# jypjypjypjyp/lvio_fusion

Hardware: AMD Instinct MI355X
Metric: local-BA iters/sec (50 KF x 10k pts) + ICP Mpairs/sec (higher is better)
Workload: dtype f64; 1 GPU; configs[3]: full sliding-window LM iteration, 50 keyframes x 10 000 landmarks (10000 TwoCamera + 71789 TwoFrame + 9629 PoseOnly + 49 IMU factors), device-resident LM loop, one independent window per GPU; n_kf=50, n_lm=10000, parallelism=1 independent windows

## Files before the change

### lvio_fusion_amd/csrc/lvf_internal.hpp

```cpp
#pragma once
#include <hip/hip_runtime.h>
#include <algorithm>
#include <cstdarg>
#include <cstdint>
#include <cstdlib>
#include <cstdio>
#include <cstring>
#include <memory>
#include <mutex>
#include <string>
#include <unordered_map>
#include <utility>
#include <vector>

#include "../../include/lvf.h"
#include "lvf_math.hpp"

namespace lvf {

void set_error(const char* fmt, ...);
int hip_fail(hipError_t e, const char* what, const char* file, int line);

#define LVF_HIP(call)                                                          \
  do {                                                                         \
// ... 356 lines not shown
  lvf::DevBuf<double> corr;
  lvf::DevBuf<char> icp_dev;
  lvf::HostPin<char> icp_host;
  lvf::DevBuf<float> create_src; lvf::HostPin<float> create_stage; hipEvent_t create_done = nullptr;
  ~lvf_scan() { if (create_done) { (void)hipEventSynchronize(create_done); (void)hipEventDestroy(create_done); } }
};

struct lvf_cloud {
  lvf_ctx* ctx = nullptr;
  int n = 0;
  lvf::DevBuf<float4> pts;
};

struct lvf_problem;
namespace lvf {
template <int CTRL>
__device__ __forceinline__ double quad_perm(double v) {
  const int lo = __builtin_amdgcn_mov_dpp(__double2loint(v), CTRL, 0xF, 0xF, true);
  const int hi = __builtin_amdgcn_mov_dpp(__double2hiint(v), CTRL, 0xF, 0xF, true);
  return __hiloint2double(hi, lo);
}
__device__ __forceinline__ double quad_sum(double v) {
  v += quad_perm<0xB1>(v);
  v += quad_perm<0x4E>(v);
  return v;
}

__device__ __forceinline__ double lane_bcast(double v, int srclane) {
  const int lo = __builtin_amdgcn_readlane(__double2loint(v), srclane);
  const int hi = __builtin_amdgcn_readlane(__double2hiint(v), srclane);
  return __hiloint2double(hi, lo);
}
__device__ __forceinline__ int wave_incl_scan(int v) {
  v += __builtin_amdgcn_update_dpp(0, v, 0x111, 0xF, 0xF, true);
  v += __builtin_amdgcn_update_dpp(0, v, 0x112, 0xF, 0xF, true);
  v += __builtin_amdgcn_update_dpp(0, v, 0x114, 0xF, 0xF, true);
  v += __builtin_amdgcn_update_dpp(0, v, 0x118, 0xF, 0xF, true);
  v += __builtin_amdgcn_update_dpp(0, v, 0x142, 0xA, 0xF, false);
  v += __builtin_amdgcn_update_dpp(0, v, 0x143, 0xC, 0xF, false);
  return v;
}
__device__ __forceinline__ double row16_sum(double v) {
  v = quad_sum(v);
  v += quad_perm<0x141>(v);
  v += quad_perm<0x140>(v);
  return v;
}
__device__ __forceinline__ double wave_sum(double v) {
  v = quad_sum(v);
  v += quad_perm<0x141>(v);
  v += quad_perm<0x140>(v);
  return (lane_bcast(v, 0) + lane_bcast(v, 16)) + (lane_bcast(v, 32) + lane_bcast(v, 48));
}
typedef unsigned lvf_v2u __attribute__((ext_vector_type(2)));
__device__ __forceinline__ void swap_halves32(double& x, double& y) {
  const lvf_v2u lo = __builtin_amdgcn_permlane32_swap((unsigned)__double2loint(x), (unsigned)__double2loint(y), false, false);
  const lvf_v2u hi = __builtin_amdgcn_permlane32_swap((unsigned)__double2hiint(x), (unsigned)__double2hiint(y), false, false);
  x = __hiloint2double((int)hi.x, (int)lo.x); y = __hiloint2double((int)hi.y, (int)lo.y);
}
__device__ __forceinline__ void swap_rows16(double& x, double& y) {
  const lvf_v2u lo = __builtin_amdgcn_permlane16_swap((unsigned)__double2loint(x), (unsigned)__double2loint(y), false, false);
  const lvf_v2u hi = __builtin_amdgcn_permlane16_swap((unsigned)__double2hiint(x), (unsigned)__double2hiint(y), false, false);
  x = __hiloint2double((int)hi.x, (int)lo.x); y = __hiloint2double((int)hi.y, (int)lo.y);
}
__device__ __forceinline__ double wave_sum32(double v[32]) {
  const int lane = threadIdx.x & 63;
#pragma unroll
  for (int i = 0; i < 16; ++i) { swap_halves32(v[i], v[i + 16]); v[i] += v[i + 16]; }
#pragma unroll
  for (int i = 0; i < 8; ++i) { swap_rows16(v[i], v[i + 8]); v[i] += v[i + 8]; }
  const bool b3 = lane & 8, b2 = lane & 4, b1 = lane & 2;
#pragma unroll
  for (int i = 0; i < 4; ++i) { const double keep = b3 ? v[i + 4] : v[i], send = b3 ? v[i] : v[i + 4]; v[i] = keep + quad_perm<0x128>(send); }
#pragma unroll
  for (int i = 0; i < 2; ++i) { const double keep = b2 ? v[i + 2] : v[i], send = b2 ? v[i] : v[i + 2]; v[i] = keep + quad_perm<0x141>(send); }
  { const double keep = b1 ? v[1] : v[0], send = b1 ? v[0] : v[1]; v[0] = keep + quad_perm<0x4E>(send); }
  return v[0] + quad_perm<0xB1>(v[0]);
}

__device__ __forceinline__ bool cell_runs(int c, int& start, int& len) {
  const int lane = threadIdx.x & 63;
  const int prev = __shfl_up(c, 1);
  const bool head = lane == 0 || c != prev;
  const unsigned long long hm = __ballot(head);
  const unsigned long long upto = (lane == 63) ? ~0ull : ((2ull << lane) - 1ull);
  start = 63 - __clzll((long long)(hm & upto));
  const unsigned long long above = hm & ~upto;
  len = (above ? __ffsll((long long)above) - 1 : 64) - lane;
  return head;
}


int problem_configure(lvf_problem* p);
}
extern "C" __attribute__((visibility("hidden"))) int lvf_problem_solve_then(lvf_problem* p, const lvf_solver_options* o, lvf_solver_summary* summary, int (*tail)(void*), void* user);
namespace lvf {
int device_sort_pairs_u32(lvf_ctx* ctx, const unsigned* keys_in, unsigned* keys_out, const int* vals_in, int* vals_out, int n, int key_bits);
struct SortP { int n, bits, db, nbins; };
constexpr int kSortMaxDigitBits = 11;
struct SortScratch { DevBuf<int> hist; DevBuf<unsigned> tkeys; DevBuf<int> tvals; };
struct SortJobDc {
  hipStream_t q; const unsigned* keys_in; unsigned* keys_out; const int* vals_in; int* vals_out; const SortP* sp; SortScratch* keep;
  const unsigned* ki; const int* vi; unsigned* ko; int* vo;
};
int device_sort_pairs_u32_dc_multi(lvf_ctx* ctx, int n_jobs, SortJobDc* jobs, int cap, int passes);
int device_scan1(lvf_ctx* ctx, const int* in, int cap, const int* n_dev, int* pos, int* total_out, const float4* pts, float4* out);
int device_scan1_on(lvf_ctx* ctx, hipStream_t q, int lane, const int* in, int cap, const int* n_dev, int* pos, int* total_out, const float4* pts, float4* out);
int side_stream(lvf_ctx* ctx, hipStream_t* out);
int enter(lvf_ctx* ctx);
const uint8_t* image_level0(const lvf_image* img, int* width, int* height, lvf_ctx** ctx);
int image_begin(const char* who, lvf_ctx* ctx, int width, int height, int max_level, lvf_image** out, uint8_t** level0);
int image_chain(lvf_image* img);
int device_exclusive_scan_i32(lvf_ctx* ctx, const int* in, int n, int* out);
int compact_points(lvf_ctx* ctx, const float4* pts, int n, const int* flags_dev, lvf_cloud** out);
struct DcTailPlan { bool supported, two_streams; int cap, passes, grid_cells, lane_ground, max_iterations, min_neighbors; float leaf, radius, thr; };
int dc_tail_begin(lvf_ctx* ctx, int cap, float resolution, float max_range, DevBuf<unsigned char>& state, std::shared_ptr<void>& keep, DcTailPlan* plan);
int dc_tail_fork(lvf_ctx* ctx, const DcTailPlan& plan, hipStream_t* q);
int dc_tail_run(lvf_ctx* ctx, const DcTailPlan& plan, hipStream_t q, const float4* surf_raw, const int* n_surf_raw, const float4* ground_raw, const int* n_ground_raw,
                unsigned long long seed, DevBuf<unsigned char>& state, std::shared_ptr<void>& keep, DevBuf<float4>& surf_out, DevBuf<float4>& ground_out);
int dc_state_bytes();
int dc_state_counts_offset();
int transform_points(lvf_ctx* ctx, const float4* in, int n, const double* pose, lvf_cloud** out);
constexpr int kDeskewFastKnots = 8;
struct DeskewRt { double R[9], t[3]; };
struct DeskewP {
  const double* knots; int n, k0, nk;
  double t_lo, t_hi, t0;
  DeskewRt E, A;
};
int deskew_prepare(const char* who, lvf_ctx* ctx, const lvf_trajectory* tr, double frame_time, const double* frame_pose7, double cycle_time, const double* extrinsic7,
// ... 40 lines not shown
```

### lvio_fusion_amd/csrc/solver_kernels.hip

```cpp
#include <hip/hip_ext.h>
#include <algorithm>
#include <chrono>
#include <cmath>
#include <cstdlib>
#include <memory>
#include <unordered_map>

#include "factor_eval.hpp"
#include "prior_eval.hpp"
#include "lvf_internal.hpp"
#include "imu_eval.hpp"

namespace lvf {
struct TfWork;
struct LmCtl;
struct Chain;
struct StageClock;
struct SpNode { int col, row_off, m, id; };
constexpr int kSpMaxLevels = 12, kSpMaxRows = 768;
struct SpLevels { int n; int first[kSpMaxLevels]; int count[kSpMaxLevels]; };
struct JacobiDev { GP<double> h0; GP<const int> frozen; };
struct SpSrc {
  GP<const double> B; int ldB, dp; GP<const double> gc; GP<const double> radius; GP<const int> rows_nat;
  GP<int> wait_counter; int wait_target; GP<int> done_counter;
// ... 217 lines not shown
                                               const uint8_t* __restrict__ pose_const, double* __restrict__ B, int ld,
                                               double* __restrict__ gc, double* __restrict__ E, int ldE,
                                               double* __restrict__ C, double* __restrict__ gr, double* __restrict__ cost) {
  __shared__ PoseD s_pose[kMaxStagedKf];
  stage_poses<kT>(s_pose, s.poses, n_kf);
  const int i = blockIdx.x * kT + threadIdx.x;
  double c = 0.0;
  if (i < n) {
    const int l = lm[i], k1 = kf1[i], k2 = kf2[i];
    const double2 a = fo[i], b = ob[i];
    const PoseD P1 = fetch_pose(s_pose, s.poses, n_kf, k1), P2 = fetch_pose(s_pose, s.poses, n_kf, k2);
    double r[2], Jd[2], L1[12], L2[12];
    if (COST_ONLY) { double J1[14], J2[14]; eval_two_frame<false>(P1, P2, left, right, a.x, a.y, b.x, b.y, s.inv_depth[l], s.w_kf[k2], r, Jd, J1, J2); }
    else eval_two_frame_local(P1, P2, left, right, a.x, a.y, b.x, b.y, s.inv_depth[l], s.w_kf[k2], r, Jd, L1, L2);
    double rho;
    const double sc = robust_scale(huber, r[0] * r[0] + r[1] * r[1], rho);
    c = 0.5 * rho;
    if (!COST_ONLY) {
      {
        const double s1 = (pose_const[k1] & 1) ? 0.0 : sc, s2 = (pose_const[k2] & 1) ? 0.0 : sc;
#pragma unroll
        for (int q = 0; q < 12; ++q) { L1[q] *= s1; L2[q] *= s2; }
      }
      const double r0 = sc * r[0], r1 = sc * r[1], d0 = sc * Jd[0], d1 = sc * Jd[1];
      atomicAdd(&C[l], d0 * d0 + d1 * d1);
      atomicAdd(&gr[l], d0 * r0 + d1 * r1);
      if (k1 == k2) {
#pragma unroll
        for (int q = 0; q < 12; ++q) L1[q] += L2[q];
        add_block66(B, ld, 6 * k1, 6 * k1, L1, L1);
#pragma unroll
        for (int q = 0; q < 6; ++q) { atomicAdd(&gc[6 * k1 + q], L1[q] * r0 + L1[6 + q] * r1); atomicAdd(&E[(size_t)l * ldE + 6 * k1 + q], L1[q] * d0 + L1[6 + q] * d1); }
      } else {
        add_block66(B, ld, 6 * k1, 6 * k1, L1, L1);
        add_block66(B, ld, 6 * k2, 6 * k2, L2, L2);
        if (k2 > k1) add_block66(B, ld, 6 * k2, 6 * k1, L2, L1); else add_block66(B, ld, 6 * k1, 6 * k2, L1, L2);
#pragma unroll
        for (int q = 0; q < 6; ++q) {
          atomicAdd(&gc[6 * k1 + q], L1[q] * r0 + L1[6 + q] * r1);
          atomicAdd(&gc[6 * k2 + q], L2[q] * r0 + L2[6 + q] * r1);
          atomicAdd(&E[(size_t)l * ldE + 6 * k1 + q], L1[q] * d0 + L1[6 + q] * d1);
          atomicAdd(&E[(size_t)l * ldE + 6 * k2 + q], L2[q] * d0 + L2[6 + q] * d1);
        }
      }
    }
  }
  block_add(c, cost);
}

struct TfWork { int first, count, k2; };
struct TfCompact { int on; GP<const int> slot; GP<double> slotB, slabP, slabQ; int staged; };
constexpr int kSlabRow = 64, kSlabQ = 32;
constexpr int kAccSlots = 63;
constexpr int kStageWave = 64 * 9 + 32;
template <bool DYN = false>
__device__ __forceinline__ void lin_tf_sorted_body(const int vb, const TfWork* __restrict__ work, int n_kf, const double2* __restrict__ fo,
                                                      const double2* __restrict__ ob, const int* __restrict__ lm,
                                                      const int* __restrict__ kf1, StateP s, CamD left, CamD right, double huber,
                                                      const uint8_t* __restrict__ pose_const, double* __restrict__ B, int ld,
                                                      double* __restrict__ gc, double* __restrict__ E, int ldE,
                                                      double* __restrict__ C, double* __restrict__ gr, double* __restrict__ cost, int unique_lk2,
                                                      unsigned long long* dbg = nullptr, const TfCompact cp = TfCompact{0, nullptr, nullptr, nullptr, nullptr, 1}, const int dbg_nw = 0) {
  __shared__ PoseD s_pose_st[DYN ? 1 : kMaxStagedKf];
  __shared__ double s_acc_st[DYN ? 1 : kMaxStagedKf * kAccSlots];
  __shared__ double s_k2_st[DYN ? 1 : 27];
  extern __shared__ double lin_lds[];
  PoseD* s_pose = DYN ? reinterpret_cast<PoseD*>(lin_lds) : s_pose_st;
  double* s_acc = DYN ? lin_lds + (sizeof(PoseD) / 8) * n_kf : s_acc_st;
  double* s_k2 = DYN ? s_acc + kAccSlots * n_kf : s_k2_st;
  double* s_stage = DYN ? s_k2 + 32 + (threadIdx.x >> 6) * kStageWave : nullptr;
  int* s_stage_k1 = reinterpret_cast<int*>(s_stage + 64 * 9);
  const TfWork w = work[vb];
  auto mark = [&](int k) { if (dbg && threadIdx.x == 0) dbg[(size_t)vb * 8 + k] = wall_clock64(); };
  unsigned long long* dbgw = dbg ? dbg + (size_t)dbg_nw * 8 + 8 + (size_t)vb * 16 + (threadIdx.x >> 6) * 4 : nullptr;
  auto markw = [&](int k) { if (dbgw && (threadIdx.x & 63) == 0) dbgw[k] = wall_clock64(); };
  mark(0);
  for (int e = threadIdx.x; e < n_kf * kAccSlots; e += kT) s_acc[e] = 0.0;
  if (threadIdx.x < 27) s_k2[threadIdx.x] = 0.0;
  stage_poses<kT>(s_pose, s.poses, n_kf);
  mark(1);
  const int k2 = w.k2;
  double c = 0.0;
  double v[27];
#pragma unroll
  for (int q = 0; q < 27; ++q) v[q] = 0.0;
  const bool active = (int)threadIdx.x < w.count;
  markw(0);
  int k1 = 0;
  double L1[12], L2[12], r0 = 0.0, r1 = 0.0;
#pragma unroll
  for (int q = 0; q < 12; ++q) { L1[q] = 0.0; L2[q] = 0.0; }
  if (active) {
    const int i = w.first + threadIdx.x;
    const int l = lm[i];
    k1 = kf1[i];
    const double2 a = fo[i], b = ob[i];
    double r[2], Jd[2];
    eval_two_frame_local(s_pose[k1], s_pose[k2], left, right, a.x, a.y, b.x, b.y, s.inv_depth[l], s.w_kf[k2], r, Jd, L1, L2);
    double rho;
    const double sc = robust_scale(huber, r[0] * r[0] + r[1] * r[1], rho);
    c = 0.5 * rho;
    {
      const double s1 = (pose_const[k1] & 1) ? 0.0 : sc, s2 = (pose_const[k2] & 1) ? 0.0 : sc;
#pragma unroll
      for (int q = 0; q < 12; ++q) { L1[q] *= s1; L2[q] *= s2; }
    }
    r0 = sc * r[0]; r1 = sc * r[1];
    const double d0 = sc * Jd[0], d1 = sc * Jd[1];
    if (cp.on) {
      double* el = E + (size_t)l * ldE + 6 * k2;
      double2* rec = reinterpret_cast<double2*>(cp.slotB + (size_t)cp.slot[i] * 8);
      double e1[6];
#pragma unroll
      for (int q = 0; q < 6; ++q) { e1[q] = L1[q] * d0 + L1[6 + q] * d1; el[q] = L2[q] * d0 + L2[6 + q] * d1; }
      rec[0] = make_double2(e1[0], e1[1]); rec[1] = make_double2(e1[2], e1[3]); rec[2] = make_double2(e1[4], e1[5]);
      rec[3] = make_double2(d0 * d0 + d1 * d1, d0 * r0 + d1 * r1);
    } else {
      atomicAdd(&C[l], d0 * d0 + d1 * d1);
      atomicAdd(&gr[l], d0 * r0 + d1 * r1);
      double* el = E + (size_t)l * ldE;
#pragma unroll
      for (int q = 0; q < 6; ++q) {
        atomicAdd(&el[6 * k1 + q], L1[q] * d0 + L1[6 + q] * d1);
        const double e2 = L2[q] * d0 + L2[6 + q] * d1;
        if (unique_lk2) el[6 * k2 + q] = e2; else atomicAdd(&el[6 * k2 + q], e2);
      }
    }
  }
  mark(2); markw(1);
  {
    {
      int q = 0;
#pragma unroll
      for (int x = 0; x < 6; ++x)
#pragma unroll
        for (int y = 0; y <= x; ++y) v[q++] = L2[x] * L2[y] + L2[6 + x] * L2[6 + y];
#pragma unroll
      for (int x = 0; x < 6; ++x) v[21 + x] = L2[x] * r0 + L2[6 + x] * r1;
    }
    const int lane = threadIdx.x & 63;
    unsigned long long remaining = __ballot(active);
    bool mine_done = !active;
    int n_groups = 0;
    for (unsigned long long rem = remaining; rem && n_groups < 5; ++n_groups)
      rem &= ~__ballot(active && k1 == __builtin_amdgcn_readlane(k1, (int)__ffsll((long long)rem) - 1));
    const int min_group = n_groups <= 4 ? 1 : 16;
    if (dbgw && lane == 0) dbgw[3] = (unsigned long long)n_groups;
#pragma unroll 1
    for (int round = 0; round < 4 && remaining; ++round) {
      const int k1u = __builtin_amdgcn_readlane(k1, (int)__ffsll((long long)remaining) - 1);
      const bool sel = active && !mine_done && k1 == k1u;
      const unsigned long long m = __ballot(sel);
      if (__popcll(m) < min_group) break;
      double* accu = s_acc + k1u * kAccSlots;
      double z = sel ? 1.0 : 0.0;
      asm volatile("" : "+v"(z));
      double M[12];
#pragma unroll
      for (int i = 0; i < 12; ++i) M[i] = L1[i] * z;
#pragma unroll
      for (int bt = 0; bt < 2; ++bt) {
        double t[32];
#pragma unroll
        for (int i = 0; i < 32; ++i) t[i] = 0.0;
        int q = 0;
#pragma unroll
        for (int x = 0; x < 6; ++x)
#pragma unroll
          for (int y = 0; y <= x; ++y) { if ((q >> 5) == bt) t[q & 31] = M[x] * L1[y] + M[6 + x] * L1[6 + y]; ++q; }
#pragma unroll
        for (int x = 0; x < 6; ++x) { if ((q >> 5) == bt) t[q & 31] = M[x] * r0 + M[6 + x] * r1; ++q; }
#pragma unroll
        for (int x = 0; x < 6; ++x)
#pragma unroll
          for (int y = 0; y < 6; ++y) { if ((q >> 5) == bt) t[q & 31] = L2[x] * M[y] + L2[6 + x] * M[6 + y]; ++q; }
        const double tot = wave_sum32(t);
        const int slot = 32 * bt + (lane >> 1);
        if (!(lane & 1) && slot < 63 && tot != 0.0) atomicAdd(&accu[slot], tot);
      }
      mine_done = mine_done || sel;
      remaining &= ~m;
    }
    if (DYN && n_groups > 4 && cp.staged) {
      double z = (active && !mine_done) ? 1.0 : 0.0;
      asm volatile("" : "+v"(z));
      double M[12];
#pragma unroll
      for (int i = 0; i < 12; ++i) M[i] = L1[i] * z;
      s_stage_k1[lane] = (active && !mine_done) ? k1 : -1;
      const int ss = lane & 7, part = lane >> 3;
      __builtin_amdgcn_fence(__ATOMIC_RELEASE, "wavefront");
      __builtin_amdgcn_wave_barrier();
      __builtin_amdgcn_fence(__ATOMIC_ACQUIRE, "wavefront");
      int kk[9];
#pragma unroll
      for (int j = 0; j < 9; ++j) kk[j] = (8 * part + j < 64) ? s_stage_k1[8 * part + j] : -2;
#pragma unroll
      for (int ch = 0; ch < 8; ++ch) {
        double t[8];
#pragma unroll
        for (int i = 0; i < 8; ++i) t[i] = 0.0;
        int q = 0;
#pragma unroll
        for (int x = 0; x < 6; ++x)
#pragma unroll
          for (int y = 0; y <= x; ++y) { if ((q >> 3) == ch) t[q & 7] = M[x] * L1[y] + M[6 + x] * L1[6 + y]; ++q; }
#pragma unroll
        for (int x = 0; x < 6; ++x) { if ((q >> 3) == ch) t[q & 7] = M[x] * r0 + M[6 + x] * r1; ++q; }
#pragma unroll
        for (int x = 0; x < 6; ++x)
#pragma unroll
          for (int y = 0; y < 6; ++y) { if ((q >> 3) == ch) t[q & 7] = L2[x] * M[y] + L2[6 + x] * M[6 + y]; ++q; }
        __builtin_amdgcn_wave_barrier();
#pragma unroll
        for (int i = 0; i < 8; ++i) s_stage[lane * 9 + i] = t[i];
        __builtin_amdgcn_fence(__ATOMIC_RELEASE, "wavefront");
        __builtin_amdgcn_wave_barrier();
        __builtin_amdgcn_fence(__ATOMIC_ACQUIRE, "wavefront");
        const int slot = 8 * ch + ss;
        double val[8];
#pragma unroll
        for (int j = 0; j < 8; ++j) val[j] = s_stage[(8 * part + j) * 9 + ss];
        double run = 0.0;
#pragma unroll
        for (int j = 0; j < 8; ++j) {
          run += val[j];
          if (j == 7 || kk[j + 1] != kk[j]) {
            if (kk[j] >= 0 && slot < kAccSlots && run != 0.0) atomicAdd(&s_acc[kk[j] * kAccSlots + slot], run);
            run = 0.0;
          }
        }
      }
    } else if (!mine_done) {
      double* acc = s_acc + k1 * kAccSlots;
      int q = 0;
#pragma unroll
      for (int x = 0; x < 6; ++x)
#pragma unroll
        for (int y = 0; y <= x; ++y) atomicAdd(&acc[q++], L1[x] * L1[y] + L1[6 + x] * L1[6 + y]);
#pragma unroll
      for (int x = 0; x < 6; ++x) atomicAdd(&acc[21 + x], L1[x] * r0 + L1[6 + x] * r1);
#pragma unroll
      for (int x = 0; x < 6; ++x)
#pragma unroll
        for (int y = 0; y < 6; ++y) atomicAdd(&acc[27 + 6 * x + y], L2[x] * L1[y] + L2[6 + x] * L1[6 + y]);
    }
  }
  mark(3); markw(2);
  {
    double v32[32];
#pragma unroll
    for (int q = 0; q < 32; ++q) v32[q] = q < 27 ? v[q] : 0.0;
    const double tot = wave_sum32(v32);
    const int lane = threadIdx.x & 63;
    if (!(lane & 1) && (lane >> 1) < 27 && tot != 0.0) atomicAdd(&s_k2[lane >> 1], tot);
  }
  block_add(c, cost);
  __syncthreads();
  mark(4);
  if (cp.on) {
    if (threadIdx.x < kSlabQ) cp.slabQ[(size_t)vb * kSlabQ + threadIdx.x] = threadIdx.x < 27 ? s_k2[threadIdx.x] : 0.0;
    double* P = cp.slabP + (size_t)vb * n_kf * kSlabRow;
    for (int e = threadIdx.x; e < k2 * kSlabRow; e += kT) {
      const int kk = e >> 6, slot = e & 63;
      P[e] = slot < kAccSlots ? s_acc[kk * kAccSlots + slot] : 0.0;
    }
  } else {
  if (threadIdx.x < 27) {
    const double val = s_k2[threadIdx.x];
    if (val != 0.0) {
      if (threadIdx.x < 21) {
        int x = 0, rem = threadIdx.x;
        while (rem > x) { rem -= x + 1; ++x; }
        atomicAdd(&B[(size_t)(6 * k2 + x) * ld + 6 * k2 + rem], val);
      } else atomicAdd(&gc[6 * k2 + threadIdx.x - 21], val);
    }
  }
  for (int e = threadIdx.x; e < n_kf * kAccSlots; e += kT) {
    const double val = s_acc[e];
    if (val == 0.0) continue;
    const int k1 = e / kAccSlots, slot = e % kAccSlots;
    if (slot < 21) {
      int x = 0, rem = slot;
      while (rem > x) { rem -= x + 1; ++x; }
      atomicAdd(&B[(size_t)(6 * k1 + x) * ld + 6 * k1 + rem], val);
    } else if (slot < 27) {
      atomicAdd(&gc[6 * k1 + slot - 21], val);
    } else {
      const int x = (slot - 27) / 6, y = (slot - 27) % 6;
      if (k2 > k1) atomicAdd(&B[(size_t)(6 * k2 + x) * ld + 6 * k1 + y], val);
      else atomicAdd(&B[(size_t)(6 * k1 + y) * ld + 6 * k2 + x], val);
    }
  }
  }
  __syncthreads();
  mark(5);
}
struct CostVisual {
  int n_tc, n_tf, n_po, g_tc, g_tf;
  GP<const double2> tc_lo, tc_ro; GP<const int> tc_lm, tc_kf; GP<const double> tc_w; CamD tc_left, tc_right;
  GP<const double2> tf_fo, tf_ob; GP<const int> tf_lm, tf_k1, tf_k2; CamD tf_left, tf_right;
  GP<const double2> po_ob; GP<const int> po_kf, po_pwi; GP<const double> po_pw; CamD po_cam;
};
struct ImuEvalArgs { int n; GP<const double> pre, sqrt_info; GP<const int> kf_i, kf_j; };
struct CostArgs {
  CostVisual a; int n_kf; StateP s; double huber; GP<double> cost; int nblocks; GP<const int> done;
  ImuEvalArgs imu; int g_imu;
  int tiles;
  ZeroList zero; int zero_wgs;
// ... 346 lines not shown
  if (tid < 64) {
    double c = tid < 15 ? 0.5 * sr[tid] * sr[tid] : 0.0;
    c = wave_sum(c);
    if (tid == 0) atomicAdd(cost + (f & (kStripes - 1)), c);
  }
  for (int e = tid; e < 30 * 30; e += kT) {
    const int a = e / 30, b = e % 30;
    const int ga = sidx[a], gb = sidx[b];
    if (gb > ga || (ga == gb && a != b)) continue;
    double h = 0.0;
#pragma unroll
    for (int k = 0; k < 15; ++k) h += sJ[k * 30 + a] * sJ[k * 30 + b];
    atomicAdd(&B[(size_t)ga * ld + gb], h);
  }
  if (tid < 30) {
    double g = 0.0;
#pragma unroll
    for (int k = 0; k < 15; ++k) g += sJ[k * 30 + tid] * sr[k];
    atomicAdd(&gc[sidx[tid]], g);
  }
  if (dbg) dbg[4] = wall_clock64();
}

struct LinVisual {
  int n_tfw, g_tc;
  GP<const TfWork> work; GP<const double2> tf_fo, tf_ob; GP<const int> tf_lm, tf_k1; CamD tf_left, tf_right; int unique_lk2; TfCompact cp;
  int n_tc; GP<const double2> tc_lo, tc_ro; GP<const int> tc_lm, tc_kf; GP<const double> tc_w; CamD tc_left, tc_right;
  int n_po, g_po; GP<const double2> po_ob; GP<const int> po_kf, po_pwi; GP<const double> po_pw; CamD po_cam;
  int n_imu; GP<const double> imu_res; ImuJ imu_J; GP<const int> imu_i, imu_j; ImuEvalArgs imu;
};
struct LinArgs {
  LinVisual v; int n_kf; StateP s; double huber; GP<const uint8_t> pose_const; GP<double> B; int ld; GP<double> gc; GP<double> E; int ldE; GP<double> C, gr, cost;
  int nblocks; GP<const int> done; GP<unsigned long long> dbg; int rows;
  GP<double> scal_reset;
  AccSel acc;
};
__device__ __forceinline__ void reset_step_scalars(double* scal) {
  for (int k = SC_COST_NEW + threadIdx.x; k < SC_N; k += kT) scal[k] = 0.0;
  if (threadIdx.x == 0) { *reinterpret_cast<int*>(scal + SC_FAIL) = 0; *reinterpret_cast<int*>(scal + SC_TICKET) = 0; }
}
__device__ __forceinline__ void lin_visual_run(const int bx, const LinArgs& A, const int set, const StateP s, double* cost) {
  const LinVisual& a = A.v;
  const int g_imu_first = a.imu.pre ? a.n_imu : 0;
  const int b = bx - g_imu_first;
  const int n_kf = A.n_kf; const double huber = A.huber; const uint8_t* pose_const = A.pose_const;
  auto pick = [set](GP<double> p0, GP<double> p1) -> double* { return (double*)(p0.p + (p1.p - p0.p) * (ptrdiff_t)set); };
  double* B = pick(A.B, A.acc.B); const int ld = A.ld; double* gc = pick(A.gc, A.acc.gc); double* E = pick(A.E, A.acc.E); const int ldE = A.ldE;
  double* C = pick(A.C, A.acc.C); double* gr = pick(A.gr, A.acc.gr);
  TfCompact cp = a.cp;
  cp.slotB = pick(a.cp.slotB, A.acc.slotB);
  if (bx < g_imu_first)
    lin_imu_eval_body(bx, a.imu, n_kf, s, pose_const, B, ld, gc, cost, A.dbg ? A.dbg + (size_t)a.n_tfw * 8 : nullptr);
  else if (b < a.n_tfw)
    lin_tf_sorted_body<true>(b, a.work, n_kf, a.tf_fo, a.tf_ob, a.tf_lm, a.tf_k1, s, a.tf_left, a.tf_right, huber, pose_const, B, ld, gc, E, ldE, C, gr, cost,
                       a.unique_lk2, A.dbg, cp, a.n_tfw);
  else if (b < a.n_tfw + a.g_tc)
    lin_tc_body<false>(b - a.n_tfw, a.n_tc, a.tc_lo, a.tc_ro, a.tc_lm, a.tc_kf, a.tc_w, s, a.tc_left, a.tc_right, huber, C, gr, cost);
  else if (b < a.n_tfw + a.g_tc + a.g_po)
    lin_po_body<false, true>(b - a.n_tfw - a.g_tc, a.n_po, n_kf, a.po_ob, a.po_kf, a.po_pwi, a.po_pw, s, a.po_cam, huber, pose_const, B, ld, gc, cost);
  else
    lin_imu_body4<true>(b - a.n_tfw - a.g_tc - a.g_po, a.n_imu, n_kf, a.imu_res, a.imu_J, a.imu_i, a.imu_j, s.poses, pose_const, B, ld, gc, cost);
}
__device__ __forceinline__ void lin_visual_body(const int bx, const LinArgs& A) {
  if (bx >= A.nblocks || (A.done && *A.done)) return;
  if (bx == 0 && A.scal_reset) reset_step_scalars(A.scal_reset);
  lin_visual_run(bx, A, 0, A.s, A.cost);
}
__global__ __launch_bounds__(kT) __attribute__((amdgpu_waves_per_eu(3))) void k_lin_visual(LinArgs a) { lin_visual_body(blockIdx.x, a); }
__global__ __launch_bounds__(kT) __attribute__((amdgpu_waves_per_eu(3))) void k_lin_visual_b(const LinArgs* __restrict__ t) { lin_visual_body(blockIdx.x, t[blockIdx.y]); }
__global__ __launch_bounds__(kT) __attribute__((amdgpu_waves_per_eu(3))) void k_lin_visual_bt(const LinArgs* __restrict__ t) { lin_visual_body(blockIdx.y, t[blockIdx.x]); }

struct TfReduceArgs {
  int n_kf, n_wg; GP<const int> run_first; GP<const double> slabP, slabQ; GP<double> B; int ld; GP<double> gc; int nblocks; GP<const int> done;
  int own_blocks; SpArgs ride;
  AccSel acc; GP<const int> pending; ZeroList stand0, stand1; int zero_wgs;
};
template <bool SEL>
__device__ __forceinline__ void tf_reduce_body(const int bx0, const TfReduceArgs& A) {
  if (bx0 >= A.nblocks) {
    const int zw = (int)bx0 - A.nblocks;
    if (SEL && zw < A.zero_wgs) {
      if (acc_set(A.acc)) zero_list_share(A.stand0, zw, A.zero_wgs);
      else zero_list_share(A.stand1, zw, A.zero_wgs);
    }
    return;
  }
  if (A.done && *A.done) return;
  if (bx0 < A.ride.nblocks) { sp_ride<SEL>(bx0, A.ride); return; }
  if (SEL && A.pending && !*A.pending) return;
  const bool s1 = acc_set_t<SEL>(A.acc) != 0;
  double* const Bs = s1 ? (double*)A.acc.B : (double*)A.B;
  double* const gcs = s1 ? (double*)A.acc.gc : (double*)A.gc;
  const int bx = bx0 - A.ride.nblocks;
  const int n_kf = A.n_kf;
  const int nchunk = (A.n_wg + 63) / 64;
  if (bx < n_kf * nchunk) {
    __shared__ double part[8][32];
    const int k = bx / nchunk, c = bx - k * nchunk, v = threadIdx.x & 31, g = threadIdx.x >> 5;
    const int r0 = A.run_first[k], r1 = A.run_first[k + 1];
    double acc = 0.0;
    if (v < 27) {
      const double* slabP = A.slabP; const double* slabQ = A.slabQ;
      double t8[8]; bool keep[8];
#pragma unroll
      for (int u = 0; u < 8; ++u) {
        const int wg = 64 * c + g + 8 * u, wgc = min(wg, A.n_wg - 1);
        const bool useP = wgc >= r1;
// ... 2669 lines not shown
  bool imu_done = false;
  const bool clean = !lin || (c.fast && p->accum_clean);
  p->accum_clean = false;
  if (p->clk && p->clk->on) (void)hipEventRecord(p->clk->ev[p->clk->rep][0], q);
  if (!clean) LVF_CHAIN_LAUNCH(p, ST_IMU_LIN, k_zero_multi, dim3(512, c.zero.count), dim3(kT), 0, q, c.zero);
  if (c.fast) {
    imu_done = true;
    stage_mark(p, ST_IMU_LIN, clean ? 0 : 1);
    LinArgs la = c.lin;
    la.huber = huber;
    if (!gated) la.done = nullptr;
    if (!iteration) la.scal_reset = nullptr;
    static const bool lin_timing = std::getenv("LVF_LIN_TIMING") != nullptr;
    if (lin_timing) { LVF_TRY(p->dbg_lin.ensure((size_t)la.v.n_tfw * 24 + 8)); la.dbg = p->dbg_lin.p; }
    static const size_t lds_pad = [] { const char* e = std::getenv("LVF_LIN_LDS_PAD"); return e ? (size_t)std::atoi(e) : (size_t)0; }();
    if (lin) LVF_CHAIN_LAUNCH(p, ST_LIN_VISUAL, k_lin_visual, dim3(la.nblocks), dim3(kT), c.lin_lds + lds_pad, q, la);
    stage_mark(p, ST_LIN_VISUAL, lin ? 1 : 0);
    if (p->compact) {
      TfReduceArgs ra = c.red;
      if (!gated) ra.done = nullptr;
      if (!iteration) { ra.nblocks = ra.own_blocks; ra.ride.nblocks = 0; }
      int zero_wgs = 0;
      if (acc) {
        ra.acc = *acc; acc_patch(ra.ride, acc);
        ra.pending = lin ? nullptr : &p->ctl.p->lin_pending;
        ra.stand0 = c.stand0; ra.stand1 = c.stand1; ra.zero_wgs = zero_wgs = kEndZeroWgs;
      }
      LVF_CHAIN_LAUNCH(p, ST_TF_REDUCE, k_tf_reduce, dim3(ra.nblocks + zero_wgs), dim3(kT), ra.ride.nblocks > 0 ? c.red_lds : 0, q, ra);
    }
    stage_mark(p, ST_TF_REDUCE, p->compact ? 1 : 0);
    if (lin_timing) {
      std::vector<unsigned long long> t((size_t)la.v.n_tfw * 8);
      LVF_HIP(hipStreamSynchronize(q));
      LVF_HIP(hipMemcpy(t.data(), p->dbg_lin.p, t.size() * 8, hipMemcpyDeviceToHost));
      double ph[5] = {0, 0, 0, 0, 0}; unsigned long long first = ~0ull, last = 0, last_start = 0;
      for (int w = 0; w < la.v.n_tfw; ++w) {
        for (int k = 0; k < 5; ++k) ph[k] += (double)(t[(size_t)w * 8 + k + 1] - t[(size_t)w * 8 + k]) * 0.01;
        first = std::min(first, t[(size_t)w * 8]); last = std::max(last, t[(size_t)w * 8 + 5]); last_start = std::max(last_start, t[(size_t)w * 8]);
      }
      {
        double mx[5] = {0, 0, 0, 0, 0}; int slow = 0; double slow_t = 0;
        for (int w = 0; w < la.v.n_tfw; ++w) {
          for (int k = 0; k < 5; ++k) mx[k] = std::max(mx[k], (double)(t[(size_t)w * 8 + k + 1] - t[(size_t)w * 8 + k]) * 0.01);
          const double tot = (double)(t[(size_t)w * 8 + 5] - t[(size_t)w * 8]) * 0.01;
          if (tot > slow_t) { slow_t = tot; slow = w; }
        }
        std::vector<TfWork> hw((size_t)la.v.n_tfw);
        LVF_HIP(hipMemcpy(hw.data(), la.v.work, hw.size() * sizeof(TfWork), hipMemcpyDeviceToHost));
        std::fprintf(stderr, "lin_tf: per-phase MAX over the workgroups (us): %.2f | %.2f | %.2f | %.2f | %.2f ; slowest workgroup %d (k2 = %d, %d blocks): %.2f us =", mx[0], mx[1], mx[2], mx[3], mx[4], slow, hw[slow].k2, hw[slow].count, slow_t);
        for (int k = 0; k < 5; ++k) std::fprintf(stderr, " %.2f", (double)(t[(size_t)slow * 8 + k + 1] - t[(size_t)slow * 8 + k]) * 0.01);
        {
          unsigned long long u[16];
          LVF_HIP(hipMemcpy(u, p->dbg_lin.p + (size_t)la.v.n_tfw * 8 + 8 + (size_t)slow * 16, sizeof(u), hipMemcpyDeviceToHost));
          std::fprintf(stderr, " ; its waves (eval us, k1-sum us, groups):");
          for (int wv = 0; wv < 4; ++wv) std::fprintf(stderr, " [%.2f %.2f %llu]", (double)(u[4 * wv + 1] - u[4 * wv]) * 0.01, (double)(u[4 * wv + 2] - u[4 * wv + 1]) * 0.01, u[4 * wv + 3]);
        }
        std::fprintf(stderr, " ; mean duration by k2 decile:");
        const int nk = la.n_kf;
        for (int dcl = 0; dcl < 5; ++dcl) {
          double sum = 0; int cnt = 0;
          for (int w = 0; w < la.v.n_tfw; ++w) if (hw[w].k2 * 5 / std::max(nk, 1) == dcl) { sum += (double)(t[(size_t)w * 8 + 5] - t[(size_t)w * 8]) * 0.01; ++cnt; }
          std::fprintf(stderr, " %.1f(%d)", cnt ? sum / cnt : 0.0, cnt);
        }
        std::fprintf(stderr, "\n");
      }
      std::fprintf(stderr, "lin_tf: the TwoFrame workgroups START within %.2f us of each other; starts of workgroups 0, 1/4, 1/2, 3/4, last (us after the first): %.2f %.2f %.2f %.2f %.2f\n", (double)(last_start - first) * 0.01,
                   (double)(t[0] - first) * 0.01, (double)(t[(size_t)(la.v.n_tfw / 4) * 8] - first) * 0.01, (double)(t[(size_t)(la.v.n_tfw / 2) * 8] - first) * 0.01,
                   (double)(t[(size_t)(3 * la.v.n_tfw / 4) * 8] - first) * 0.01, (double)(t[(size_t)(la.v.n_tfw - 1) * 8] - first) * 0.01);
      std::fprintf(stderr, "lin_tf phases (us, mean over %d workgroups): stage %.2f | eval+landmark atomics %.2f | k1 sums %.2f | k2 sums %.2f | flush %.2f ; first start -> last end %.2f\n",
                   la.v.n_tfw, ph[0] / la.v.n_tfw, ph[1] / la.v.n_tfw, ph[2] / la.v.n_tfw, ph[3] / la.v.n_tfw, ph[4] / la.v.n_tfw, (double)(last - first) * 0.01);
      if (la.v.imu.pre) {
        unsigned long long u[5];
        LVF_HIP(hipMemcpy(u, p->dbg_lin.p + (size_t)la.v.n_tfw * 8, sizeof(u), hipMemcpyDeviceToHost));
        std::fprintf(stderr, "lin_imu phases of factor 0 (us): stage %.2f | raw residual + pre-weighting Jacobian (one lane) %.2f | weight + to tangent %.2f | J^T J, J^T r %.2f ; start %.2f after the first TwoFrame workgroup, end %.2f before the last one's end\n",
                     (double)(u[1] - u[0]) * 0.01, (double)(u[2] - u[1]) * 0.01, (double)(u[3] - u[2]) * 0.01, (double)(u[4] - u[3]) * 0.01, ((double)u[0] - (double)first) * 0.01, ((double)last - (double)u[4]) * 0.01);
      }
    }
  } else {
    if (p->tc && p->tc->n)
      hipLaunchKernelGGL(k_lin_tc<false>, dim3(grid(p->tc->n)), dim3(kT), 0, q, p->tc->n, (const double2*)p->tc->ob_a.p, (const double2*)p->tc->ob_b.p,
                         p->tc->idx_a.p, p->tc->idx_b.p, p->tc->wblk.n ? p->tc->wblk.p : (const double*)nullptr, s, p->tc->cam_a, p->tc->cam_b, huber, p->C.p, p->gr.p, cost);
    if (p->tf && p->tf->n)
      hipLaunchKernelGGL(k_lin_tf<false>, dim3(grid(p->tf->n)), dim3(kT), 0, q, p->tf->n, p->n_kf, (const double2*)p->tf->ob_a.p, (const double2*)p->tf->ob_b.p,
                         p->tf->idx_a.p, p->tf->idx_b.p, p->tf->idx_c.p, s, p->tf->cam_a, p->tf->cam_b, huber, p->pose_const.p, p->B.p, p->dpad,
                         p->gc.p, p->E.p, p->ldE, p->C.p, p->gr.p, cost);
    if (p->po && p->po->n)
      hipLaunchKernelGGL(k_lin_po<false>, dim3(grid(p->po->n)), dim3(kT), 0, q, p->po->n, p->n_kf, (const double2*)p->po->ob_a.p, p->po->idx_a.p,
                         p->po->idx_b.p, p->po->table.p, s, p->po->cam_a, huber, p->pose_const.p, p->B.p, p->dpad, p->gc.p, cost);
  }
  if (c.has_imu && !imu_done) {
    LVF_TRY(launch_imu(p->imu, p->st, true));
    ImuJ J;
    for (int k = 0; k < 8; ++k) J.j[k] = p->imu->jac[k].p;
    hipLaunchKernelGGL(k_lin_imu, dim3(p->imu->n), dim3(64), 0, q, p->imu->n, p->n_kf, p->imu->res.p, J, p->imu->idx_a.p, p->imu->idx_b.p,
                       p->st->poses.p, p->pose_const.p, p->B.p, p->dpad, p->gc.p, cost);
  }
  if (c.has_prior) {
    const lvf_batch* pb = p->prior;
    const PriorArgs P{pb->n, pb->idx_a.p, pb->idx_b.p, pb->table.p, pb->ob_a.p, pb->ob_b.p};
    hipLaunchKernelGGL(k_prior_lin, dim3((pb->n + 63) / 64), dim3(64), 0, q, P, p->st->poses.p, p->pose_const.p, p->B.p, p->dpad, p->gc.p, cost);
  }
  LVF_HIP(hipGetLastError());
  p->linearized = true;
  return LVF_OK;
}

static int await_band_work(lvf_problem* p) {
  if (!p->band_pending) return LVF_OK;
  LVF_HIP(hipEventSynchronize(p->ev_band));
  p->band_pending = false;
  p->n_band_work = p->h_n_band_work[0];
  if (p->chain && p->chain->merged_level0) {
    SchurSp0Args& a = p->chain->ssp0;
    a.n_work = p->n_band_work;
    a.nblocks = a.n_work + a.sp.nblocks + a.sp_b.nblocks + a.sp_c.nblocks;
  }
  return LVF_OK;
}

static int enqueue_reduced_system(lvf_problem* p, const double* radius_dev, bool reset_scalars, bool gated, bool* level0_done, const AccSel* acc = nullptr) {
  hipStream_t q = p->ctx->stream;
  const Chain& c = *p->chain;
// ... 1199 lines not shown
```

Baseline: 5676 iter/s.

## Compute TwoFrame per-keyframe Gram sums with f64 MFMA instead of wave reductions

```diff
diff --git a/lvio_fusion_amd/csrc/lvf_internal.hpp b/lvio_fusion_amd/csrc/lvf_internal.hpp
--- a/lvio_fusion_amd/csrc/lvf_internal.hpp
+++ b/lvio_fusion_amd/csrc/lvf_internal.hpp
@@ -432,30 +432,25 @@
   v += quad_perm<0x140>(v);
   return (lane_bcast(v, 0) + lane_bcast(v, 16)) + (lane_bcast(v, 32) + lane_bcast(v, 48));
 }
-typedef unsigned lvf_v2u __attribute__((ext_vector_type(2)));
-__device__ __forceinline__ void swap_halves32(double& x, double& y) {
-  const lvf_v2u lo = __builtin_amdgcn_permlane32_swap((unsigned)__double2loint(x), (unsigned)__double2loint(y), false, false);
-  const lvf_v2u hi = __builtin_amdgcn_permlane32_swap((unsigned)__double2hiint(x), (unsigned)__double2hiint(y), false, false);
-  x = __hiloint2double((int)hi.x, (int)lo.x); y = __hiloint2double((int)hi.y, (int)lo.y);
-}
-__device__ __forceinline__ void swap_rows16(double& x, double& y) {
-  const lvf_v2u lo = __builtin_amdgcn_permlane16_swap((unsigned)__double2loint(x), (unsigned)__double2loint(y), false, false);
-  const lvf_v2u hi = __builtin_amdgcn_permlane16_swap((unsigned)__double2hiint(x), (unsigned)__double2hiint(y), false, false);
-  x = __hiloint2double((int)hi.x, (int)lo.x); y = __hiloint2double((int)hi.y, (int)lo.y);
-}
-__device__ __forceinline__ double wave_sum32(double v[32]) {
+typedef double lvf_d4 __attribute__((ext_vector_type(4)));
+constexpr int kGramCols = 13, kGramRow = 14, kGramLane = 30;
+constexpr int kGramTile = 16 * kGramLane;
+__device__ __forceinline__ void gram_stage(double* tile, const int quarter, const double (&j0)[kGramRow], const double (&j1)[kGramRow]) {
   const int lane = threadIdx.x & 63;
+  __builtin_amdgcn_wave_barrier();
+  if ((lane >> 4) == quarter) {
+    double2* d = reinterpret_cast<double2*>(tile + (lane & 15) * kGramLane);
 #pragma unroll
-  for (int i = 0; i < 16; ++i) { swap_halves32(v[i], v[i + 16]); v[i] += v[i + 16]; }
-#pragma unroll
-  for (int i = 0; i < 8; ++i) { swap_rows16(v[i], v[i + 8]); v[i] += v[i + 8]; }
-  const bool b3 = lane & 8, b2 = lane & 4, b1 = lane & 2;
-#pragma unroll
-  for (int i = 0; i < 4; ++i) { const double keep = b3 ? v[i + 4] : v[i], send = b3 ? v[i] : v[i + 4]; v[i] = keep + quad_perm<0x128>(send); }
-#pragma unroll
-  for (int i = 0; i < 2; ++i) { const double keep = b2 ? v[i + 2] : v[i], send = b2 ? v[i] : v[i + 2]; v[i] = keep + quad_perm<0x141>(send); }
-  { const double keep = b1 ? v[1] : v[0], send = b1 ? v[0] : v[1]; v[0] = keep + quad_perm<0x4E>(send); }
-  return v[0] + quad_perm<0xB1>(v[0]);
+    for (int q = 0; q < kGramRow / 2; ++q) { d[q] = make_double2(j0[2 * q], j0[2 * q + 1]); d[kGramRow / 2 + q] = make_double2(j1[2 * q], j1[2 * q + 1]); }
+  }
+  __builtin_amdgcn_fence(__ATOMIC_RELEASE, "wavefront");
+  __builtin_amdgcn_wave_barrier();
+  __builtin_amdgcn_fence(__ATOMIC_ACQUIRE, "wavefront");
+}
+__device__ __forceinline__ double gram_operand(const double* tile, const int t) {
+  const int lane = threadIdx.x & 63, c = lane & 15, k = lane >> 4;
+  const double x = tile[(2 * t + (k >> 1)) * kGramLane + (k & 1) * kGramRow + min(c, kGramCols - 1)];
+  return c < kGramCols ? x : 0.0;
 }
 
 __device__ __forceinline__ bool cell_runs(int c, int& start, int& len) {
diff --git a/lvio_fusion_amd/csrc/solver_kernels.hip b/lvio_fusion_amd/csrc/solver_kernels.hip
--- a/lvio_fusion_amd/csrc/solver_kernels.hip
+++ b/lvio_fusion_amd/csrc/solver_kernels.hip
@@ -293,8 +293,12 @@
 struct TfCompact { int on; GP<const int> slot; GP<double> slotB, slabP, slabQ; int staged; };
 constexpr int kSlabRow = 64, kSlabQ = 32;
 constexpr int kAccSlots = 63;
-constexpr int kStageWave = 64 * 9 + 32;
-template <bool DYN = false>
+constexpr int kStageWave = kGramTile;
+__device__ __forceinline__ int gram_slot_k2(const int i, const int j) { return i >= 6 ? -1 : j <= i ? i * (i + 1) / 2 + j : j == 12 ? 21 + i : -1; }
+__device__ __forceinline__ int gram_slot_k1(const int i, const int j) {
+  const int y = i - 6;
+  return (y < 0 || y >= 6) ? -1 : j < 6 ? 27 + 6 * j + y : j < 12 ? (j - 6 <= y ? y * (y + 1) / 2 + j - 6 : -1) : j == 12 ? 21 + y : -1;
+}
 __device__ __forceinline__ void lin_tf_sorted_body(const int vb, const TfWork* __restrict__ work, int n_kf, const double2* __restrict__ fo,
                                                       const double2* __restrict__ ob, const int* __restrict__ lm,
                                                       const int* __restrict__ kf1, StateP s, CamD left, CamD right, double huber,
@@ -302,15 +306,11 @@
                                                       double* __restrict__ gc, double* __restrict__ E, int ldE,
                                                       double* __restrict__ C, double* __restrict__ gr, double* __restrict__ cost, int unique_lk2,
                                                       unsigned long long* dbg = nullptr, const TfCompact cp = TfCompact{0, nullptr, nullptr, nullptr, nullptr, 1}, const int dbg_nw = 0) {
-  __shared__ PoseD s_pose_st[DYN ? 1 : kMaxStagedKf];
-  __shared__ double s_acc_st[DYN ? 1 : kMaxStagedKf * kAccSlots];
-  __shared__ double s_k2_st[DYN ? 1 : 27];
   extern __shared__ double lin_lds[];
-  PoseD* s_pose = DYN ? reinterpret_cast<PoseD*>(lin_lds) : s_pose_st;
-  double* s_acc = DYN ? lin_lds + (sizeof(PoseD) / 8) * n_kf : s_acc_st;
-  double* s_k2 = DYN ? s_acc + kAccSlots * n_kf : s_k2_st;
-  double* s_stage = DYN ? s_k2 + 32 + (threadIdx.x >> 6) * kStageWave : nullptr;
-  int* s_stage_k1 = reinterpret_cast<int*>(s_stage + 64 * 9);
+  PoseD* s_pose = reinterpret_cast<PoseD*>(lin_lds);
+  double* s_acc = lin_lds + (sizeof(PoseD) / 8) * n_kf;
+  double* s_k2 = s_acc + kAccSlots * n_kf;
+  double* s_stage = s_k2 + 32 + (threadIdx.x >> 6) * kStageWave;
   const TfWork w = work[vb];
   auto mark = [&](int k) { if (dbg && threadIdx.x == 0) dbg[(size_t)vb * 8 + k] = wall_clock64(); };
   unsigned long long* dbgw = dbg ? dbg + (size_t)dbg_nw * 8 + 8 + (size_t)vb * 16 + (threadIdx.x >> 6) * 4 : nullptr;
@@ -322,9 +322,6 @@
   mark(1);
   const int k2 = w.k2;
   double c = 0.0;
-  double v[27];
-#pragma unroll
-  for (int q = 0; q < 27; ++q) v[q] = 0.0;
   const bool active = (int)threadIdx.x < w.count;
   markw(0);
   int k1 = 0;
@@ -370,132 +367,65 @@
   }
   mark(2); markw(1);
   {
-    {
+    const int lane = threadIdx.x & 63, col = lane & 15, rq = lane >> 4;
+    const int n_act = __popcll(__ballot(active));
+    const int k1_prev = __shfl_up(k1, 1);
+    const unsigned long long heads = cp.staged ? __ballot(active && (lane == 0 || k1 != k1_prev)) : 1ull;
+    if (dbgw && lane == 0) dbgw[3] = (unsigned long long)__popcll(heads);
+    const int slot_k2a = gram_slot_k2(rq, col), slot_k2b = gram_slot_k2(4 + rq, col);
+    const int slot_k1a = cp.staged ? gram_slot_k1(4 + rq, col) : -1, slot_k1b = cp.staged ? gram_slot_k1(8 + rq, col) : -1;
+    const bool second_l1 = lane >= 32 && col >= 6 && col < 12;
+    const double j0[kGramRow] = {L2[0], L2[1], L2[2], L2[3], L2[4], L2[5], L1[0], L1[1], L1[2], L1[3], L1[4], L1[5], r0, 0.0};
+    const double j1[kGramRow] = {L2[6], L2[7], L2[8], L2[9], L2[10], L2[11], L1[6], L1[7], L1[8], L1[9], L1[10], L1[11], r1, 0.0};
+    lvf_d4 acc = {0.0, 0.0, 0.0, 0.0};
+    auto flush_run = [&](const int last) {
+      double* accu = s_acc + __builtin_amdgcn_readlane(k1, last) * kAccSlots;
+      if (slot_k1a >= 0) atomicAdd(&accu[slot_k1a], acc[1]);
+      if (slot_k1b >= 0) atomicAdd(&accu[slot_k1b], acc[2]);
+      if (lane >= 32) acc[1] = 0.0;
+      acc[2] = 0.0;
+    };
+#pragma unroll 1
+    for (int qt = 0; qt < 4 && 16 * qt < n_act; ++qt) {
+      gram_stage(s_stage, qt, j0, j1);
+      double x[8];
+#pragma unroll
+      for (int t = 0; t < 8; ++t) x[t] = gram_operand(s_stage, t);
+#pragma unroll
+      for (int t = 0; t < 8; ++t) {
+        const int l0 = 16 * qt + 2 * t;
+        if (l0 >= n_act) break;
+        const unsigned hb = (unsigned)(heads >> l0) & 3u;
+        if ((hb & 1u) && l0 > 0) flush_run(l0 - 1);
+        const bool split = hb & 2u;
+        acc = __builtin_amdgcn_mfma_f64_16x16x4f64((split && second_l1) ? 0.0 : x[t], x[t], acc, 0, 0, 0);
+        if (split) {
+          flush_run(l0);
+          acc = __builtin_amdgcn_mfma_f64_16x16x4f64(second_l1 ? x[t] : 0.0, x[t], acc, 0, 0, 0);
+        }
+      }
+    }
+    if (n_act > 0) {
+      flush_run(n_act - 1);
+      if (slot_k2a >= 0) atomicAdd(&s_k2[slot_k2a], acc[0]);
+      if (slot_k2b >= 0) atomicAdd(&s_k2[slot_k2b], acc[1]);
+    }
+    if (!cp.staged && active) {
+      double* accl = s_acc + k1 * kAccSlots;
       int q = 0;
 #pragma unroll
       for (int x = 0; x < 6; ++x)
 #pragma unroll
-        for (int y = 0; y <= x; ++y) v[q++] = L2[x] * L2[y] + L2[6 + x] * L2[6 + y];
-#pragma unroll
-      for (int x = 0; x < 6; ++x) v[21 + x] = L2[x] * r0 + L2[6 + x] * r1;
-    }
-    const int lane = threadIdx.x & 63;
-    unsigned long long remaining = __ballot(active);
-    bool mine_done = !active;
-    int n_groups = 0;
-    for (unsigned long long rem = remaining; rem && n_groups < 5; ++n_groups)
-      rem &= ~__ballot(active && k1 == __builtin_amdgcn_readlane(k1, (int)__ffsll((long long)rem) - 1));
-    const int min_group = n_groups <= 4 ? 1 : 16;
-    if (dbgw && lane == 0) dbgw[3] = (unsigned long long)n_groups;
-#pragma unroll 1
-    for (int round = 0; round < 4 && remaining; ++round) {
-      const int k1u = __builtin_amdgcn_readlane(k1, (int)__ffsll((long long)remaining) - 1);
-      const bool sel = active && !mine_done && k1 == k1u;
-      const unsigned long long m = __ballot(sel);
-      if (__popcll(m) < min_group) break;
-      double* accu = s_acc + k1u * kAccSlots;
-      double z = sel ? 1.0 : 0.0;
-      asm volatile("" : "+v"(z));
-      double M[12];
-#pragma unroll
-      for (int i = 0; i < 12; ++i) M[i] = L1[i] * z;
-#pragma unroll
-      for (int bt = 0; bt < 2; ++bt) {
-        double t[32];
-#pragma unroll
-        for (int i = 0; i < 32; ++i) t[i] = 0.0;
-        int q = 0;
-#pragma unroll
-        for (int x = 0; x < 6; ++x)
-#pragma unroll
-          for (int y = 0; y <= x; ++y) { if ((q >> 5) == bt) t[q & 31] = M[x] * L1[y] + M[6 + x] * L1[6 + y]; ++q; }
-#pragma unroll
-        for (int x = 0; x < 6; ++x) { if ((q >> 5) == bt) t[q & 31] = M[x] * r0 + M[6 + x] * r1; ++q; }
-#pragma unroll
-        for (int x = 0; x < 6; ++x)
-#pragma unroll
-          for (int y = 0; y < 6; ++y) { if ((q >> 5) == bt) t[q & 31] = L2[x] * M[y] + L2[6 + x] * M[6 + y]; ++q; }
-        const double tot = wave_sum32(t);
-        const int slot = 32 * bt + (lane >> 1);
-        if (!(lane & 1) && slot < 63 && tot != 0.0) atomicAdd(&accu[slot], tot);
-      }
-      mine_done = mine_done || sel;
-      remaining &= ~m;
-    }
-    if (DYN && n_groups > 4 && cp.staged) {
-      double z = (active && !mine_done) ? 1.0 : 0.0;
-      asm volatile("" : "+v"(z));
-      double M[12];
-#pragma unroll
-      for (int i = 0; i < 12; ++i) M[i] = L1[i] * z;
-      s_stage_k1[lane] = (active && !mine_done) ? k1 : -1;
-      const int ss = lane & 7, part = lane >> 3;
-      __builtin_amdgcn_fence(__ATOMIC_RELEASE, "wavefront");
-      __builtin_amdgcn_wave_barrier();
-      __builtin_amdgcn_fence(__ATOMIC_ACQUIRE, "wavefront");
-      int kk[9];
-#pragma unroll
-      for (int j = 0; j < 9; ++j) kk[j] = (8 * part + j < 64) ? s_stage_k1[8 * part + j] : -2;
-#pragma unroll
-      for (int ch = 0; ch < 8; ++ch) {
-        double t[8];
-#pragma unroll
-        for (int i = 0; i < 8; ++i) t[i] = 0.0;
-        int q = 0;
-#pragma unroll
-        for (int x = 0; x < 6; ++x)
-#pragma unroll
-          for (int y = 0; y <= x; ++y) { if ((q >> 3) == ch) t[q & 7] = M[x] * L1[y] + M[6 + x] * L1[6 + y]; ++q; }
-#pragma unroll
-        for (int x = 0; x < 6; ++x) { if ((q >> 3) == ch) t[q & 7] = M[x] * r0 + M[6 + x] * r1; ++q; }
-#pragma unroll
-        for (int x = 0; x < 6; ++x)
-#pragma unroll
-          for (int y = 0; y < 6; ++y) { if ((q >> 3) == ch) t[q & 7] = L2[x] * M[y] + L2[6 + x] * M[6 + y]; ++q; }
-        __builtin_amdgcn_wave_barrier();
-#pragma unroll
-        for (int i = 0; i < 8; ++i) s_stage[lane * 9 + i] = t[i];
-        __builtin_amdgcn_fence(__ATOMIC_RELEASE, "wavefront");
-        __builtin_amdgcn_wave_barrier();
-        __builtin_amdgcn_fence(__ATOMIC_ACQUIRE, "wavefront");
-        const int slot = 8 * ch + ss;
-        double val[8];
-#pragma unroll
-        for (int j = 0; j < 8; ++j) val[j] = s_stage[(8 * part + j) * 9 + ss];
-        double run = 0.0;
-#pragma unroll
-        for (int j = 0; j < 8; ++j) {
-          run += val[j];
-          if (j == 7 || kk[j + 1] != kk[j]) {
-            if (kk[j] >= 0 && slot < kAccSlots && run != 0.0) atomicAdd(&s_acc[kk[j] * kAccSlots + slot], run);
-            run = 0.0;
-          }
-        }
-      }
-    } else if (!mine_done) {
-      double* acc = s_acc + k1 * kAccSlots;
-      int q = 0;
+        for (int y = 0; y <= x; ++y) atomicAdd(&accl[q++], L1[x] * L1[y] + L1[6 + x] * L1[6 + y]);
+#pragma unroll
+      for (int x = 0; x < 6; ++x) atomicAdd(&accl[21 + x], L1[x] * r0 + L1[6 + x] * r1);
 #pragma unroll
       for (int x = 0; x < 6; ++x)
 #pragma unroll
-        for (int y = 0; y <= x; ++y) atomicAdd(&acc[q++], L1[x] * L1[y] + L1[6 + x] * L1[6 + y]);
-#pragma unroll
-      for (int x = 0; x < 6; ++x) atomicAdd(&acc[21 + x], L1[x] * r0 + L1[6 + x] * r1);
-#pragma unroll
-      for (int x = 0; x < 6; ++x)
-#pragma unroll
-        for (int y = 0; y < 6; ++y) atomicAdd(&acc[27 + 6 * x + y], L2[x] * L1[y] + L2[6 + x] * L1[6 + y]);
+        for (int y = 0; y < 6; ++y) atomicAdd(&accl[27 + 6 * x + y], L2[x] * L1[y] + L2[6 + x] * L1[6 + y]);
     }
   }
   mark(3); markw(2);
-  {
-    double v32[32];
-#pragma unroll
-    for (int q = 0; q < 32; ++q) v32[q] = q < 27 ? v[q] : 0.0;
-    const double tot = wave_sum32(v32);
-    const int lane = threadIdx.x & 63;
-    if (!(lane & 1) && (lane >> 1) < 27 && tot != 0.0) atomicAdd(&s_k2[lane >> 1], tot);
-  }
   block_add(c, cost);
   __syncthreads();
   mark(4);
@@ -948,7 +878,7 @@
   if (bx < g_imu_first)
     lin_imu_eval_body(bx, a.imu, n_kf, s, pose_const, B, ld, gc, cost, A.dbg ? A.dbg + (size_t)a.n_tfw * 8 : nullptr);
   else if (b < a.n_tfw)
-    lin_tf_sorted_body<true>(b, a.work, n_kf, a.tf_fo, a.tf_ob, a.tf_lm, a.tf_k1, s, a.tf_left, a.tf_right, huber, pose_const, B, ld, gc, E, ldE, C, gr, cost,
+    lin_tf_sorted_body(b, a.work, n_kf, a.tf_fo, a.tf_ob, a.tf_lm, a.tf_k1, s, a.tf_left, a.tf_right, huber, pose_const, B, ld, gc, E, ldE, C, gr, cost,
                        a.unique_lk2, A.dbg, cp, a.n_tfw);
   else if (b < a.n_tfw + a.g_tc)
     lin_tc_body<false>(b - a.n_tfw, a.n_tc, a.tc_lo, a.tc_ro, a.tc_lm, a.tc_kf, a.tc_w, s, a.tc_left, a.tc_right, huber, C, gr, cost);
@@ -3724,7 +3654,7 @@
         {
           unsigned long long u[16];
           LVF_HIP(hipMemcpy(u, p->dbg_lin.p + (size_t)la.v.n_tfw * 8 + 8 + (size_t)slow * 16, sizeof(u), hipMemcpyDeviceToHost));
-          std::fprintf(stderr, " ; its waves (eval us, k1-sum us, groups):");
+          std::fprintf(stderr, " ; its waves (eval us, Gram sums us, first-keyframe runs):");
           for (int wv = 0; wv < 4; ++wv) std::fprintf(stderr, " [%.2f %.2f %llu]", (double)(u[4 * wv + 1] - u[4 * wv]) * 0.01, (double)(u[4 * wv + 2] - u[4 * wv + 1]) * 0.01, u[4 * wv + 3]);
         }
         std::fprintf(stderr, " ; mean duration by k2 decile:");
@@ -3739,7 +3669,7 @@
       std::fprintf(stderr, "lin_tf: the TwoFrame workgroups START within %.2f us of each other; starts of workgroups 0, 1/4, 1/2, 3/4, last (us after the first): %.2f %.2f %.2f %.2f %.2f\n", (double)(last_start - first) * 0.01,
                    (double)(t[0] - first) * 0.01, (double)(t[(size_t)(la.v.n_tfw / 4) * 8] - first) * 0.01, (double)(t[(size_t)(la.v.n_tfw / 2) * 8] - first) * 0.01,
                    (double)(t[(size_t)(3 * la.v.n_tfw / 4) * 8] - first) * 0.01, (double)(t[(size_t)(la.v.n_tfw - 1) * 8] - first) * 0.01);
-      std::fprintf(stderr, "lin_tf phases (us, mean over %d workgroups): stage %.2f | eval+landmark atomics %.2f | k1 sums %.2f | k2 sums %.2f | flush %.2f ; first start -> last end %.2f\n",
+      std::fprintf(stderr, "lin_tf phases (us, mean over %d workgroups): stage %.2f | eval+landmark atomics %.2f | k1 + k2 sums (one Gram product) %.2f | cost sum + barrier %.2f | flush %.2f ; first start -> last end %.2f\n",
                    la.v.n_tfw, ph[0] / la.v.n_tfw, ph[1] / la.v.n_tfw, ph[2] / la.v.n_tfw, ph[3] / la.v.n_tfw, ph[4] / la.v.n_tfw, (double)(last - first) * 0.01);
       if (la.v.imu.pre) {
         unsigned long long u[5];
```

After: 5634 iter/s. About the same (-0.7%).
